# sriram-0311/MC-SLAM

Measured on AMD Instinct MI355X. Metric: multi-cam frames/sec (4-cam 1280x720 @2000 kpts/cam, extract + intra-rig match), higher is better.
Workload: dtype u8; 1 GPU; 4-cam rig 1280x720, 2000 kpts/cam, extract + all-pairs intra-rig match (configs[1]); slots=4, frames_per_launch=128, cameras=4, nfeatures=2000

## Files before the change

### mc-slam_amd/csrc/mcorb_kernels.hip

```cpp
#include <hip/hip_runtime.h>
#include <stdint.h>
#include <string.h>
#include <vector>

#include "mcorb_common.h"
#include "mcorb_device.h"
#include "mcorb_kernels.h"

namespace mcorb {

constexpr int kResizeRows = kResizeTileH;

template <int NF>
__global__ __launch_bounds__(256) void k_resize(uint8_t *__restrict__ pyr, Geom g, int level,
                                                const ResizeTap *__restrict__ tabs, int srcPitch, int srcRows)
{
    extern __shared__ __attribute__((aligned(16))) uint8_t win[];
    const LevelGeom &D = g.lv[level];
    const LevelGeom &S = g.lv[level - 1];
    const int img = blockIdx.z;
    uint8_t *base = pyr + (size_t)img * g.imgBytes;
    const int tid = threadIdx.x;
    const int bx0 = blockIdx.x * 256, by0 = blockIdx.y * kResizeRows;
    const int bx1 = min(bx0 + 255, D.w - 1), by1 = min(by0 + kResizeRows - 1, D.h - 1);
    const int sx0 = tabs[D.xtab + bx0].s0 & ~15, sx1 = tabs[D.xtab + bx1].s1;
    const int sy0 = tabs[D.ytab + by0].s0, sy1 = tabs[D.ytab + by1].s1;
    const int nq = ((sx1 - sx0) >> 4) + 1, nr = sy1 - sy0 + 1;
    const int wave = wave_uniform(tid >> 6);
    const int wy0 = by0 + wave * (kResizeRows / 4);
    uint2 ytap;
    {
        const int l = tid & 63;
        const int dy = min(wy0 + (l < kResizeRows / 4 ? l : 0), D.h - 1);
        ytap = *reinterpret_cast<const uint2 *>(tabs + D.ytab + dy);
    }
    const int dx4 = bx0 + (tid & 63) * 4;
    const int dxc = min(dx4, ((D.w + 3) & ~3) - 4);
    const uint4 t01 = *reinterpret_cast<const uint4 *>(tabs + D.xtab + dxc);
    const uint4 t23 = *reinterpret_cast<const uint4 *>(tabs + D.xtab + dxc + 2);
    {
        const uint8_t *sp = base + S.off + (size_t)sy0 * S.pitch + sx0;
        uint4 *w128 = reinterpret_cast<uint4 *>(win);
        const int pq = srcPitch >> 4;
        const float rcp_pq = 1.0f / (float)pq;
        if constexpr (NF > 0) {
            uint4 v[NF];
            bool ok[NF];
#pragma unroll
            for (int k = 0; k < NF; k++) {
                const int i = tid + 256 * k, ic = min(i, nr * pq - 1);
                const int r = (int)(((float)ic + 0.5f) * rcp_pq), q = ic - r * pq;
                ok[k] = i < nr * pq && q < nq;
                v[k] = *reinterpret_cast<const uint4 *>(sp + (size_t)r * S.pitch + 16 * min(q, nq - 1));
            }
            const int spare = (srcPitch >> 4) * srcRows;
#pragma unroll
            for (int k = 0; k < NF; k++) w128[ok[k] ? tid + 256 * k : spare] = v[k];
        } else {
            for (int i = tid; i < nr * pq; i += 256) {
                const int r = (int)(((float)i + 0.5f) * rcp_pq), q = i - r * pq;
                if (q < nq) w128[i] = *reinterpret_cast<const uint4 *>(sp + (size_t)r * S.pitch + 16 * q);
            }
        }
    }
    __syncthreads();
    asm volatile("" ::"v"(ytap.x), "v"(ytap.y), "v"(t01.x), "v"(t01.y), "v"(t01.z), "v"(t01.w), "v"(t23.x), "v"(t23.y), "v"(t23.z), "v"(t23.w));
    if (dx4 >= D.w) return;
    const uint32_t tw[8] = {t01.x, t01.y, t01.z, t01.w, t23.x, t23.y, t23.z, t23.w};
    int s0[4], s1[4], a0[4], a1[4];
#pragma unroll
    for (int k = 0; k < 4; k++) {
        s0[k] = (int)(tw[2 * k] & 0xffff) - sx0;
        s1[k] = (int)(tw[2 * k] >> 16) - sx0;
        a0[k] = (int)(short)(tw[2 * k + 1] & 0xffff);
        a1[k] = (int)(short)(tw[2 * k + 1] >> 16);
    }
    const uint32_t mask = dx4 + 4 > D.w ? 0xffffffffu >> (8 * (dx4 + 4 - D.w)) : 0xffffffffu;
    int rowA = -1, rowB = -1;
    uint32_t HA[4], HB[4];
    const uint32_t ldsWin = (uint32_t)(uintptr_t)(__attribute__((address_space(3))) void *)win;
    uint32_t sb[4];
#pragma unroll
    for (int k = 0; k < 4; k++) sb[k] = ldsWin + (uint32_t)s0[k];
    auto hrow = [&](int sr, uint32_t *Hout) {
        const uint32_t ro = (uint32_t)__mul24(sr - sy0, srcPitch);
        const uint32_t ad0 = sb[0] + ro, ad1 = sb[1] + ro, ad2 = sb[2] + ro, ad3 = sb[3] + ro;
        uint32_t x0, x1, x2, x3, x4, x5, x6, x7;
        asm volatile("ds_read_u8 %0, %8\n\tds_read_u8 %1, %8 offset:1\n\t"
                     "ds_read_u8 %2, %9\n\tds_read_u8 %3, %9 offset:1\n\t"
                     "ds_read_u8 %4, %10\n\tds_read_u8 %5, %10 offset:1\n\t"
                     "ds_read_u8 %6, %11\n\tds_read_u8 %7, %11 offset:1\n\t"
                     "s_waitcnt lgkmcnt(0)"
                     : "=&v"(x0), "=&v"(x1), "=&v"(x2), "=&v"(x3), "=&v"(x4), "=&v"(x5), "=&v"(x6), "=&v"(x7)
                     : "v"(ad0), "v"(ad1), "v"(ad2), "v"(ad3)
                     : "memory");
        Hout[0] = (__umul24(x0, (uint32_t)a0[0]) + __umul24(x1, (uint32_t)a1[0])) >> 4;
        Hout[1] = (__umul24(x2, (uint32_t)a0[1]) + __umul24(x3, (uint32_t)a1[1])) >> 4;
        Hout[2] = (__umul24(x4, (uint32_t)a0[2]) + __umul24(x5, (uint32_t)a1[2])) >> 4;
        Hout[3] = (__umul24(x6, (uint32_t)a0[3]) + __umul24(x7, (uint32_t)a1[3])) >> 4;
    };
#pragma unroll
    for (int rr = 0; rr < kResizeRows / 4; rr++) {
        const int dy = wy0 + rr;
        if (dy >= D.h) break;
        const uint32_t ys = (uint32_t)__builtin_amdgcn_readlane((int)ytap.x, rr), yc = (uint32_t)__builtin_amdgcn_readlane((int)ytap.y, rr);
        const int r0 = (int)(ys & 0xffff), r1 = (int)(ys >> 16);
        if (r0 != rowA) {
            if (r0 == rowB) {
#pragma unroll
                for (int k = 0; k < 4; k++) HA[k] = HB[k];
            } else {
                hrow(r0, HA);
            }
            rowA = r0;
        }
        if (r1 != rowB) {
            if (r1 == rowA) {
#pragma unroll
                for (int k = 0; k < 4; k++) HB[k] = HA[k];
            } else {
                hrow(r1, HB);
            }
            rowB = r1;
        }
        const uint32_t b0 = yc & 0xffff, b1 = yc >> 16;
        uint32_t p0[4], p1[4];
#pragma unroll
        for (int k = 0; k < 4; k++) {
            p0[k] = __umul24(b0, HA[k]) + 0x20000u;
            p1[k] = __umul24(b1, HB[k]);
        }
        uint32_t t01v, t23v;
        asm("v_add_u32_sdwa %0, %1, %2 dst_sel:DWORD dst_unused:UNUSED_PAD src0_sel:WORD_1 src1_sel:WORD_1" : "=v"(t01v) : "v"(p0[0]), "v"(p1[0]));
        asm("v_add_u32_sdwa %0, %1, %2 dst_sel:WORD_1 dst_unused:UNUSED_PRESERVE src0_sel:WORD_1 src1_sel:WORD_1" : "+v"(t01v) : "v"(p0[1]), "v"(p1[1]));
        asm("v_add_u32_sdwa %0, %1, %2 dst_sel:DWORD dst_unused:UNUSED_PAD src0_sel:WORD_1 src1_sel:WORD_1" : "=v"(t23v) : "v"(p0[2]), "v"(p1[2]));
        asm("v_add_u32_sdwa %0, %1, %2 dst_sel:WORD_1 dst_unused:UNUSED_PRESERVE src0_sel:WORD_1 src1_sel:WORD_1" : "+v"(t23v) : "v"(p0[3]), "v"(p1[3]));
        const u16x2 s01 = __builtin_bit_cast(u16x2, t01v) >> (unsigned short)2, s23 = __builtin_bit_cast(u16x2, t23v) >> (unsigned short)2;
        const uint32_t out = __builtin_amdgcn_perm(__builtin_bit_cast(uint32_t, s23), __builtin_bit_cast(uint32_t, s01), 0x06040200u);
        *reinterpret_cast<uint32_t *>(base + D.off + (size_t)dy * D.pitch + dx4) = out & mask;
    }
}


struct FastCell {
    int on;
    int cell;
    int ph;
    int wi, hi;
    int rows;
    int g0, ng;
    int R;
    float rcp_ng;
    uint32_t headMask, tailMask;
    uint32_t org;
    const uint8_t *src;
    int pitch;
};

constexpr int kFastCellRecDw = 8;
__device__ __forceinline__ void fast_cell_setup(const uint8_t *pyr, const Geom &g, int img, int cell, const uint32_t *__restrict__ rec, FastCell &C)
{
    const uint4 r = *reinterpret_cast<const uint4 *>(rec + (size_t)cell * kFastCellRecDw);
    const uint2 r4 = *reinterpret_cast<const uint2 *>(rec + (size_t)cell * kFastCellRecDw + 4);
    C.cell = cell;
    C.src = pyr + (size_t)img * g.imgBytes + r.x;
    C.org = r.y;
    C.pitch = (int)r.z;
    C.rows = (int)(r.w & 0xff);
    C.wi = (int)((r.w >> 8) & 0xff);
    C.hi = (int)((r.w >> 16) & 0xff);
    C.on = (int)((r.w >> 24) & 1);
    C.ph = (int)((r.w >> 25) & 3);
    C.g0 = (int)(r4.x & 0xff);
    C.ng = (int)((r4.x >> 8) & 0xff);
    C.R = (int)(r4.x >> 16);
    C.rcp_ng = __uint_as_float(r4.y);
    const uint2 r6 = *reinterpret_cast<const uint2 *>(rec + (size_t)cell * kFastCellRecDw + 6);
    C.headMask = r6.x;
    C.tailMask = r6.y;
}

int fast_cell_table(const Geom &g, std::vector<uint32_t> &tab)
{
    const int off = (int)tab.size();
    tab.resize(tab.size() + (size_t)g.cells * kFastCellRecDw, 0u);
    for (int level = 0; level < g.nlevels; level++) {
        const LevelGeom &L = g.lv[level];
        for (int cl = 0; cl < L.nCols * L.nRows; cl++) {
            const int ci = cl / L.nCols, cj = cl - ci * L.nCols;
            const int iniY = kMinBorder + ci * L.hCell;
            int maxY = iniY + L.hCell + 6;
            const int iniX = kMinBorder + cj * L.wCell;
            int maxX = iniX + L.wCell + 6;
            const bool skip = (iniY >= L.maxBorderY - 3) || (iniX >= L.maxBorderX - 6);
            if (maxY > L.maxBorderY) maxY = L.maxBorderY;
            if (maxX > L.maxBorderX) maxX = L.maxBorderX;
            const int cols = maxX - iniX, rows = maxY - iniY;
            const int wi = cols - 6, hi = rows - 6;
            const int ph = iniX & 3, g0 = (ph + 3) >> 2;
            const bool on = !(skip || wi <= 0 || hi <= 0);
            const int ng = on ? ((ph + 2 + wi) >> 2) - g0 + 1 : 1;
            uint32_t *r = tab.data() + off + (size_t)(L.cell0 + cl) * kFastCellRecDw;
            r[0] = on ? (uint32_t)(L.off + (size_t)iniY * L.pitch + (iniX - ph)) : 0u;
            r[1] = ((uint32_t)(ci * L.hCell) << 20) + ((uint32_t)(cj * L.wCell - ph) << 8);
            r[2] = (uint32_t)L.pitch;
            r[3] = on ? ((uint32_t)rows | ((uint32_t)wi << 8) | ((uint32_t)hi << 16) | (1u << 24) | ((uint32_t)ph << 25)) : 0u;
            r[4] = (uint32_t)g0 | ((uint32_t)ng << 8) | ((uint32_t)(64 / ng) << 16);
            const float rcp = 1.0f / (float)ng;
            uint32_t bits;
            memcpy(&bits, &rcp, 4);
            r[5] = bits;
            auto pxmask = [&](int G) {
                static const uint32_t bit[4] = {1u << 15, 1u, 1u << 31, 1u << 16};
                uint32_t m = 0;
                for (int j = 0; j < 4; j++) {
                    const int x = 4 * G + j - (ph + 3);
                    if (x >= 0 && x < wi) m |= bit[j];
                }
                return m;
            };
            r[6] = on ? pxmask(g0) : 0u;
            r[7] = on ? pxmask(g0 + ng - 1) : 0u;
        }
    }
    return off;
}

constexpr int kFastListCap = 768;

#define EMAX __builtin_elementwise_max
#define EMIN __builtin_elementwise_min
struct FastLane {
    int off0;
    uint32_t vmask;
};
template <int TP>
__device__ __forceinline__ FastLane fast_lane_setup(const FastCell &C, int lane)
{
    FastLane L;
    const int r = (int)(((float)lane + 0.5f) * C.rcp_ng);
    const int gi = lane - r * C.ng;
    const bool act = r < C.R;
    L.off0 = act ? (3 + r) * TP + 4 * (C.g0 + gi) : 3 * TP + 4 * C.g0;
    uint32_t m = 0x80018001u;
    m = gi == 0 ? m & C.headMask : m;
    m = gi == C.ng - 1 ? m & C.tailMask : m;
    L.vmask = act ? m : 0u;
    return L;
}

template <int TP>
__device__ __forceinline__ int fast_pass1(const uint8_t *tile, uint32_t *glist, const FastCell &C, int T, int lane, int &row0, int gcap,
                                          const FastLane &L)
{
    const u16x2 Tev = u16x2{(unsigned short)T, (unsigned short)T};
    const u16x2 Tod = u16x2{(unsigned short)(256 * T + 255), (unsigned short)(256 * T + 255)};
    int nG = 0;
    auto trip = [&](int rb, bool tail) {
        int off = L.off0 + rb * TP;
        bool in = true;
        if (tail) {
            in = (int)(((float)lane + 0.5f) * C.rcp_ng) + rb < C.hi;
            off = in ? off : 3 * TP + 4 * C.g0;
        }
        const uint32_t *p = reinterpret_cast<const uint32_t *>(tile + off);
        const uint32_t Cc = p[0], Cl = p[-1], Cr = p[1], Up = p[-3 * (TP / 4)], Dn = p[3 * (TP / 4)];
        const uint32_t Lf = __builtin_amdgcn_alignbyte(Cc, Cl, 1);
        const uint32_t Rt = __builtin_amdgcn_alignbyte(Cr, Cc, 3);
#define U16(X) __builtin_bit_cast(u16x2, (uint32_t)(X))
#define S16(X) __builtin_bit_cast(s16x2, (uint32_t)(X))
        const u16x2 hO = EMIN(EMAX(U16(Up), U16(Dn)), EMAX(U16(Lf), U16(Rt)));
        const u16x2 lO = EMAX(EMIN(U16(Up), U16(Dn)), EMIN(U16(Lf), U16(Rt)));
        const u16x2 hOm = U16(__builtin_bit_cast(uint32_t, hO) & 0xff00ff00u), lOm = U16(__builtin_bit_cast(uint32_t, lO) & 0xff00ff00u);
        const u16x2 vO = U16(Cc & 0xff00ff00u);
        const u16x2 wO = EMAX(__builtin_elementwise_sub_sat(hOm, vO), __builtin_elementwise_sub_sat(vO, lOm));
        const uint32_t zO = __builtin_bit_cast(uint32_t, __builtin_elementwise_sub_sat(wO, Tod));
        const s16x2 vE = S16(Cc & 0x00ff00ffu), uE = S16(Up & 0x00ff00ffu), dE = S16(Dn & 0x00ff00ffu);
        const s16x2 lE = S16(Lf & 0x00ff00ffu), rE = S16(Rt & 0x00ff00ffu);
        const s16x2 wE = EMAX(EMIN(EMAX(uE, dE), EMAX(lE, rE)) - vE, vE - EMAX(EMIN(uE, dE), EMIN(lE, rE)));
        const uint32_t sE = __builtin_bit_cast(uint32_t, __builtin_bit_cast(s16x2, Tev) - wE);
#undef U16
#undef S16
        const uint32_t M = ((sE & 0x80008000u) | (zO & 0x00010001u)) & L.vmask;
        const bool c = M != 0 && in;
        const unsigned long long b = __builtin_amdgcn_ballot_w64(c);
        if (c) glist[lane_rank(b, nG)] = M | ((uint32_t)off >> 1);
        nG += __popcll(b);
    };
    int rb = row0;
    for (; rb + C.R <= C.hi && nG + 64 <= gcap; rb += C.R) trip(rb, false);
    if (rb < C.hi && rb + C.R > C.hi && nG + 64 <= gcap) {
        trip(rb, true);
        rb += C.R;
    }
    row0 = rb;
    return nG;
}

__device__ __forceinline__ int fast_expand(const uint32_t *glist, uint16_t *work, int nG, int lane)
{
    int nA = 0;
    for (int i0 = 0; i0 < nG; i0 += 64) {
        const bool in = i0 + lane < nG;
        const uint32_t E = in ? glist[i0 + lane] : 0u;
        const uint32_t m = E & 0x80018001u;
        const int n1 = in ? __popc(m) - 1 : 0;
        const unsigned long long b0 = __builtin_amdgcn_ballot_w64((n1 & 1) != 0), b1 = __builtin_amdgcn_ballot_w64(n1 >= 2);
        int o = nA + lane + lane_rank(b0) + 2 * lane_rank(b1);
        const uint32_t off = (E & 0x3ffeu) << 1;
        asm volatile("" ::: "memory");
        if (m & 0x8000u) work[o++] = (uint16_t)off;
        if (m & 0x1u) work[o++] = (uint16_t)(off + 1);
        if (m & 0x80000000u) work[o++] = (uint16_t)(off + 2);
        if (m & 0x10000u) work[o++] = (uint16_t)(off + 3);
        const int cnt = min(nG - i0, 64);
        nA += cnt + __popcll(b0) + 2 * __popcll(b1);
        asm volatile("" ::: "memory");
    }
    return nA;
}

template <int TP>
__device__ __forceinline__ int fast_arc_score(const uint8_t *tile, int pos)
{
    int lo = pos - (3 * TP + 3);
    asm volatile("" : "+v"(lo));
    const uint8_t *c = tile + lo + (3 * TP + 3);
    u16x2 X[8];
    X[0] = u16x2{c[3 * TP], c[-3 * TP]};          X[1] = u16x2{c[3 * TP + 1], c[-3 * TP - 1]};
    X[2] = u16x2{c[2 * TP + 2], c[-2 * TP - 2]};  X[3] = u16x2{c[TP + 3], c[-TP - 3]};
    X[4] = u16x2{c[3], c[-3]};                    X[5] = u16x2{c[-TP + 3], c[TP - 3]};
    X[6] = u16x2{c[-2 * TP + 2], c[2 * TP - 2]};  X[7] = u16x2{c[-3 * TP + 1], c[3 * TP - 1]};
    const uint32_t v = c[0];
    u16x2 Sn[8], Sx[8], Pn[8], Px[8];
    Sn[7] = Sx[7] = X[7];
    Pn[0] = Px[0] = X[0];
#pragma unroll
    for (int i = 6; i >= 1; i--) { Sn[i] = EMIN(X[i], Sn[i + 1]); Sx[i] = EMAX(X[i], Sx[i + 1]); }
#pragma unroll
    for (int i = 1; i < 8; i++) { Pn[i] = EMIN(X[i], Pn[i - 1]); Px[i] = EMAX(X[i], Px[i - 1]); }
    Sn[0] = Pn[7]; Sx[0] = Px[7];
    u16x2 bn, bx;
#pragma unroll
    for (int k = 0; k < 8; k++) {
        const u16x2 wn = EMIN(Sn[k], __builtin_shufflevector(Pn[k], Pn[k], 1, 0));
        const u16x2 wx = EMAX(Sx[k], __builtin_shufflevector(Px[k], Px[k], 1, 0));
        bn = k ? EMAX(bn, wn) : wn;
        bx = k ? EMIN(bx, wx) : wx;
    }
    const int Mx = max((int)bn.x, (int)bn.y), Mn = min((int)bx.x, (int)bx.y);
    const int a = max(Mx - (int)v, (int)v - Mn);
    return a < 0 ? 0 : a;
}
#undef EMAX
#undef EMIN

template <int TP>
__global__ __launch_bounds__(64) void k_fast_cells(const uint8_t *__restrict__ pyr, Geom g, int iniTh, int minTh,
                                                   int tileB, int scB, int cap, const uint32_t *__restrict__ cellRec,
                                                   uint32_t *__restrict__ cell_kp, int *__restrict__ cell_cnt)
{
    extern __shared__ __attribute__((aligned(16))) uint8_t lds[];
    constexpr int NQ = TP / 16;
    uint8_t *tile = lds + 16;
    uint8_t *sc = tile + tileB + 16;
    uint8_t *sc2 = sc - 2 * TP;
    uint16_t *work = reinterpret_cast<uint16_t *>(sc + scB + 16);
    uint32_t *glist = reinterpret_cast<uint32_t *>(work + cap / 2);
    const int gcap = cap >> 2;
    struct __attribute__((packed, aligned(4))) Chunk { uint32_t a, b, c, d; };

    const int lane = threadIdx.x;
    const int img = blockIdx.y;
    FastCell C;
    fast_cell_setup(pyr, g, img, wave_uniform(xcd_remap(blockIdx.x, gridDim.x)), cellRec, C);
    int *out_cnt = cell_cnt + (size_t)img * g.cells + C.cell;
    if (!C.on) {
        if (lane == 0) *out_cnt = 0;
        return;
    }

    FastLane FL;
    for (int r = lane; r < C.rows; r += 64) {
        Chunk ch[NQ];
#pragma unroll
        for (int q = 0; q < NQ; q++) ch[q] = *reinterpret_cast<const Chunk *>(C.src + (size_t)r * C.pitch + 16 * q);
        uint4 *dst = reinterpret_cast<uint4 *>(tile + r * TP);
#pragma unroll
        for (int q = 0; q < NQ; q++) dst[q] = uint4{ch[q].a, ch[q].b, ch[q].c, ch[q].d};
    }
    {
        uint4 *s128 = reinterpret_cast<uint4 *>(sc);
        for (int i = lane; i < scB / 16; i += 64) s128[i] = uint4{0, 0, 0, 0};
        FL = fast_lane_setup<TP>(C, lane);
    }
    __syncthreads();

    uint32_t *dst = cell_kp + ((size_t)img * g.cells + C.cell) * g.cellCap;
    int total = 0;
    auto score = [&](int nA, int T) {
        for (int i = lane; i < nA; i += 64) {
            const int pos = work[i];
            const int a = fast_arc_score<TP>(tile, pos);
            sc2[pos] = (uint8_t)(a > T ? a : 0);
        }
    };
    auto nms = [&](int nA) {
        for (int i0 = 0; i0 < nA; i0 += 64) {
            const int i = i0 + lane;
            const int pos = i < nA ? (int)work[i] : 3 * TP;
            int lo = pos - (TP + 1);
            asm volatile("" : "+v"(lo));
            const uint8_t *s = sc2 + lo + (TP + 1);
            const uint32_t a = s[0];
            const uint32_t n = max(max(max((uint32_t)s[1], (uint32_t)s[-1]), max((uint32_t)s[-TP - 1], (uint32_t)s[-TP])),
                                   max(max((uint32_t)s[-TP + 1], (uint32_t)s[TP - 1]), max((uint32_t)s[TP], (uint32_t)s[TP + 1])));
            const bool keep = a > n;
            const unsigned long long b = __builtin_amdgcn_ballot_w64(keep);
            if (keep) {
                const int o = lane_rank(b, total);
                const int yy = (int)(((float)pos + 0.5f) * (1.0f / (float)TP)), xx = __mul24(yy, -TP) + pos;
                if (o < g.cellCap) dst[o] = C.org + ((uint32_t)yy << 20) + ((uint32_t)xx << 8) + (a - 1);
            }
            total += __popcll(b);
        }
    };
    int T = iniTh;
#pragma unroll 1
    for (int attempt = 0; attempt < 2; attempt++) {
        int row0 = 0, sweep = 0;
#pragma unroll 1
        for (;;) {
            const bool whole = row0 == 0;
            const int nG = fast_pass1<TP>(tile, glist, C, T, lane, row0, gcap, FL);
            __syncthreads();
            const int nA = fast_expand(glist, work, nG, lane);
            __syncthreads();
            if (sweep == 0) {
                score(nA, T);
                __syncthreads();
            }
            if (sweep == 1 || (whole && row0 >= C.hi)) nms(nA);
            if (row0 >= C.hi) {
                if (sweep == 1 || whole) break;
                sweep = 1;
                row0 = 0;
            }
            __syncthreads();
        }
        if (total || T == minTh) break;
        T = minTh;
        __syncthreads();
    }
    if (lane == 0) *out_cnt = total;
}

constexpr int kCompactCopies = 4;
template <int kCompactWaves>
__device__ __forceinline__ int block_exclusive_scan(int v, int *wsum, int *total)
{
    const int lane = threadIdx.x & 63, wave = threadIdx.x >> 6;
    int s = v;
#pragma unroll
    for (int o = 1; o < 64; o <<= 1) {
        const int t = __shfl_up(s, o);
        if (lane >= o) s += t;
    }
    if (lane == 63) wsum[wave] = s;
    __syncthreads();
    if (wave == 0) {
        const int w = lane < kCompactWaves ? wsum[lane] : 0;
        int t = w;
#pragma unroll
        for (int o = 1; o < kCompactWaves; o <<= 1) {
            const int u = __shfl_up(t, o);
            if (lane >= o) t += u;
        }
        if (lane < kCompactWaves) wsum[lane] = t - w;
        if (lane == kCompactWaves - 1) *total = t;
    }
    __syncthreads();
    return wsum[wave] + s - v;
}

template <int kCompactWG, int kCompactCells, int NC>
__global__ __launch_bounds__(kCompactWG, 8) void k_compact(const uint32_t *__restrict__ cell_kp, const int *__restrict__ cell_cnt,
                                                        Geom g, const uint16_t *__restrict__ lut, uint32_t *__restrict__ sorted_dev,
                                                        uint32_t *__restrict__ cand, int *__restrict__ tbl,
                                                        int *__restrict__ overflow, int bktCap, int cellsCap)
{
    extern __shared__ __attribute__((aligned(16))) int sh[];
    int *hist = sh;
    uint32_t *bkey = reinterpret_cast<uint32_t *>(hist + NC * bktCap);
    uint16_t *cnts = reinterpret_cast<uint16_t *>(hist + 2 * NC * bktCap);
    constexpr int kCompactWaves = kCompactWG / 64;
    __shared__ int wsum[kCompactWaves];
    __shared__ int s_tot, s_base, s_nz;
    const int tid = threadIdx.x, lane = tid & 63, wave = tid >> 6;
    const int level = blockIdx.y, img = blockIdx.x;
    const LevelGeom &L = g.lv[level];
    const int nc = L.nCols * L.nRows;
    const int *cnt = cell_cnt + (size_t)img * g.cells;
    const int cap = g.cellCap;
    const int B = L.nBuckets;
    const int W0 = L.maxBorderX - kMinBorder, H0 = L.maxBorderY - kMinBorder;
    uint16_t *tx = cnts + cellsCap, *ty = tx + W0;

    int s = 0, t = 0, over = 0;
    for (int c = tid; c < L.cell0; c += kCompactWG) { const int v = cnt[c]; s += v < cap ? v : cap; }
    for (int c = tid; c < nc; c += kCompactWG) {
        int v = cnt[L.cell0 + c];
        if (v > cap) { v = cap; over = 1; }
        cnts[c] = (uint16_t)v;
        t += v;
    }
    for (int c = nc + tid; c < min(nc + 2 * kCompactCells, cellsCap); c += kCompactWG) cnts[c] = 0;
    for (int i = tid; i < W0 + H0; i += kCompactWG) tx[i] = lut[L.lutx + i];
    (void)block_exclusive_scan<kCompactWaves>(s, wsum, &s_base);
    (void)block_exclusive_scan<kCompactWaves>(t, wsum, &s_tot);
    const int base = s_base, T = s_tot;
    for (int b = tid; b < NC * (B + 1); b += kCompactWG) { hist[b] = 0; bkey[b] = 0; }
    int *tb = tbl + (size_t)img * tbl_ints(g.bucketTotal);
    if (tid == 0) {
        s_nz = 0;
        tb[kTblLvlOff + level] = base;
        if (level == g.nlevels - 1) tb[kTblLvlOff + g.nlevels] = base + T;
        if (base + T > g.candCap) over = 1;
    }
    if (over) atomicOr(overflow, 1);
    __syncthreads();

    const uint32_t *src = cell_kp + ((size_t)img * g.cells + L.cell0) * cap;
    const int wave_u = wave_uniform(wave);
    auto walk = [&](auto &&fn) {
        static_assert(kCompactCells == 8 || kCompactCells == 4 || kCompactCells == 2, "the counts are read as one 4-, 8- or 16-byte word");
        constexpr int step = kCompactWaves * kCompactCells;
        const int ncUp = (nc + kCompactCells - 1) & ~(kCompactCells - 1);
        auto load = [&](int c0, int *n, uint32_t *p) {
            if constexpr (kCompactCells == 8) {
                const uint4 q = *reinterpret_cast<const uint4 *>(cnts + c0);
                n[0] = q.x & 0xffff; n[1] = q.x >> 16; n[2] = q.y & 0xffff; n[3] = q.y >> 16;
                n[4] = q.z & 0xffff; n[5] = q.z >> 16; n[6] = q.w & 0xffff; n[7] = q.w >> 16;
            } else if constexpr (kCompactCells == 4) {
                const uint2 q = *reinterpret_cast<const uint2 *>(cnts + c0);
                n[0] = q.x & 0xffff; n[1] = q.x >> 16; n[2] = q.y & 0xffff; n[3] = q.y >> 16;
            } else {
                const uint32_t q = *reinterpret_cast<const uint32_t *>(cnts + c0);
                n[0] = q & 0xffff; n[1] = q >> 16;
            }
#pragma unroll
            for (int u = 0; u < kCompactCells; u++) {
                const uint32_t *cb = src + (size_t)min(c0 + u, nc - 1) * cap;
                p[u] = cb[min(lane, max(n[u], 1) - 1)];
            }
        };
        auto run = [&](int c0, const int *n, const uint32_t *p) {
            int big = 0;
#pragma unroll
            for (int u = 0; u < kCompactCells; u++) {
                big |= n[u];
                if (lane < n[u]) fn(p[u], (c0 + u) * cap + lane);
            }
            if (big > 64) {
#pragma unroll
                for (int u = 0; u < kCompactCells; u++)
                    for (int k = lane + 64; k < n[u]; k += 64) fn(src[(size_t)(c0 + u) * cap + k], (c0 + u) * cap + k);
            }
        };
        int c0 = wave_u * kCompactCells;
        if (c0 >= nc) return;
        int nA[kCompactCells], nB[kCompactCells];
        uint32_t pA[kCompactCells], pB[kCompactCells];
        load(c0, nA, pA);
        while (true) {
            load(min(c0 + step, ncUp), nB, pB);
            run(c0, nA, pA);
            c0 += step;
            if (c0 >= nc) break;
            load(min(c0 + step, ncUp), nA, pA);
            run(c0, nB, pB);
            c0 += step;
            if (c0 >= nc) break;
        }
    };
    walk([&](uint32_t p, int order) {
        const uint32_t code = (uint32_t)tx[cand_x(p)] | (uint32_t)ty[cand_y(p)];
        const uint32_t key = ((uint32_t)cand_resp(p) << 23) | (uint32_t)(kPickOrderMask - order);
        const int slot = (int)code * NC + (lane & (NC - 1));
        atomicAdd(&hist[slot], 1);
        atomicMax(&bkey[slot], key);
    });
    __syncthreads();
    {
        const int bper = (B + kCompactWG - 1) / kCompactWG;
        const int b0 = tid * bper;
        int bs = 0, nzl = 0;
        for (int k = 0; k < bper; k++)
            if (b0 + k < B) {
                int v = 0;
#pragma unroll
                for (int c = 0; c < NC; c++) v += hist[(b0 + k) * NC + c];
                bs += v;
                nzl += v > 0;
            }
        if (nzl) atomicAdd(&s_nz, nzl);
        int brun = block_exclusive_scan<kCompactWaves>(bs, wsum, &s_tot);
        for (int k = 0; k < bper; k++) {
            if (b0 + k < B) {
#pragma unroll
                for (int c = 0; c < NC; c++) { const int v = hist[(b0 + k) * NC + c]; hist[(b0 + k) * NC + c] = brun; brun += v; }
            }
        }
        if (tid == 0) hist[B * NC] = T;
    }
    __syncthreads();
    int *bs_out = tb + kTblHead + L.bucket0;
    for (int b = tid; b <= B; b += kCompactWG) bs_out[b] = hist[b * NC];
    __syncthreads();
    uint32_t *sd = sorted_dev + (size_t)img * g.candCap + base;
    const int room = g.candCap - base;
// ... 452 lines not shown
constexpr int kTileU4 = 4 * 64;
static_assert(32 * kKnnQT * kKnnWaves == kKnnQueriesPerBlock, "the host reads the accepted-pair lists in blocks of kKnnQueriesPerBlock queries");
static_assert(kTileU4 * 16 == 32 * kKnnExpandBytes, "k_expand's tile and the scratch size the engine allocates");

__global__ __launch_bounds__(256) void k_expand(const uint8_t *__restrict__ desc, const int *__restrict__ counts,
                                                const int *__restrict__ setmap, int kcap, uint4 *__restrict__ E,
                                                int *__restrict__ lcounts)
{
    const int i = blockIdx.y;
    const int src = setmap ? setmap[i] : i;
    const int n = min(max(counts[src], 0), kcap);
    if (blockIdx.x == 0 && threadIdx.x == 0) lcounts[i] = n;
    const int d = blockIdx.x * 256 + threadIdx.x;
    if (d >= n) return;
    const uint4 *dp = reinterpret_cast<const uint4 *>(desc + ((size_t)src * kcap + d) * 32);
    const uint4 lo = dp[0], hi = dp[1];
    const uint32_t w[8] = {lo.x, lo.y, lo.z, lo.w, hi.x, hi.y, hi.z, hi.w};
    uint4 *out = E + ((size_t)i * (kcap / 32) + (d >> 5)) * kTileU4 + (d & 31);
#pragma unroll
    for (int sh = 0; sh < 8; sh++) {
        uint32_t o[4];
#pragma unroll
        for (int q = 0; q < 4; q++) {
            uint32_t x = (w[sh] >> (8 * q)) & 0xffu;
            x = (x | (x << 12)) & 0x000f000fu;
            x = (x | (x << 6)) & 0x03030303u;
            x = (x | (x << 3)) & 0x11111111u;
            o[q] = (x << 3) | 0x22222222u;
        }
        out[(sh >> 1) * 64 + (sh & 1) * 32] = uint4{o[0], o[1], o[2], o[3]};
    }
}

template <int kKnnStageTiles, int kWavesPerSimd, bool FOLD>
__global__ __launch_bounds__(64 * kKnnWaves, kWavesPerSimd) void k_knn2(const uint4 *__restrict__ E, const int *__restrict__ lcounts,
                                                           const int2 *__restrict__ pairs, int kcap, int nchunks, int npairs,
                                                           int qblocks, uint2 *__restrict__ part, int chunkLen,
                                                           float dist_thresh, float ratio, KnnRow *__restrict__ rows,
                                                           uint32_t *__restrict__ mlist, int *__restrict__ mcount)
{
    __shared__ __attribute__((aligned(16))) uint4 stage[2 * kKnnStageTiles * kTileU4 + 2 * 64];
    const int tid = threadIdx.x, lane = tid & 63, wave = tid >> 6, half = lane >> 5;
    const int slot = blockIdx.x >> 3, grp = slot / qblocks;
    const int unit = grp * 8 + (blockIdx.x & 7);
    if (unit >= npairs * nchunks) return;
    const int pair = unit / nchunks, chunk = unit - pair * nchunks;
    const int2 qt = pairs[pair];
    const int nq = lcounts[qt.x], nt = lcounts[qt.y];
    const int qbi = slot - grp * qblocks;
    const int qb = qbi * kKnnQueriesPerBlock;
    if (qb >= nq) {
        if (FOLD && tid == 0) mcount[pair * qblocks + qbi] = 0;
        return;
    }
    const int t0 = chunk * chunkLen;
    const int tn = min(nt - t0, chunkLen);
    const int tilesPerSet = kcap / 32;
    const int ntiles = tn > 0 ? (tn + 31) >> 5 : 0;
    const float kNone = -__builtin_inff();
    float k0[kKnnQT], k1[kKnnQT];
#pragma unroll
    for (int u = 0; u < kKnnQT; u++) k0[u] = k1[u] = kNone;

    if (tn > 0) {
        const int qtile0 = (qb >> 5) + wave * kKnnQT;
        v4i Bf[kKnnQT][4];
#pragma unroll
        for (int u = 0; u < kKnnQT; u++) {
            const int tq = min(qtile0 + u, tilesPerSet - 1);
            const uint4 *src = E + ((size_t)qt.x * tilesPerSet + tq) * kTileU4 + lane;
#pragma unroll
            for (int s = 0; s < 4; s++) Bf[u][s] = __builtin_bit_cast(v4i, src[s * 64]);
        }
        v16f Crow;
#pragma unroll
        for (int e = 0; e < 16; e++) Crow[e] = (float)(31 - ((e & 3) + 8 * (e >> 2) + 4 * half));
        const uint4 *Et = E + ((size_t)qt.y * tilesPerSet + (t0 >> 5)) * kTileU4;
        const int nstage = (ntiles + kKnnStageTiles - 1) / kKnnStageTiles;
        static_assert(kTileU4 == 64 * kKnnWaves, "one LDS-DMA round of the workgroup = one tile (wave w moves K-step w)");
        auto fill = [&](int st, int buf) {
#pragma unroll
            for (int k = 0; k < kKnnStageTiles; k++) {
                const int e0 = k * kTileU4 + wave * 64;
                if (st * kKnnStageTiles + k < ntiles)
                    __builtin_amdgcn_global_load_lds((const __attribute__((address_space(1))) void *)(Et + (size_t)st * kKnnStageTiles * kTileU4 + e0 + lane),
                                                     (__attribute__((address_space(3))) void *)(&stage[buf * kKnnStageTiles * kTileU4 + e0]), 16, 0, 0);
            }
        };
        fill(0, 0);
        asm volatile("s_waitcnt vmcnt(0)" ::: "memory");
        __syncthreads();
        auto fold2 = [&](int u, float x, float y) {
            const float t = __builtin_amdgcn_fmed3f(k0[u], x, y);
            k0[u] = __builtin_fmaxf(__builtin_fmaxf(k0[u], x), y);
            k1[u] = __builtin_fmaxf(k1[u], t);
        };
        auto raise = [&]() {
#pragma unroll
            for (int u = 0; u < kKnnQT; u++) { k0[u] += 32.0f; k1[u] += 32.0f; }
        };
        auto top2 = [&](const v16f (&acc)[kKnnQT]) {
            raise();
#pragma unroll
            for (int u = 0; u < kKnnQT; u++)
#pragma unroll
                for (int e = 0; e < 16; e += 2) fold2(u, acc[u][e], acc[u][e + 1]);
        };
        constexpr int kSc = 0x85858585;
        v4i Af[4];
        auto tile = [&](const int base, const uint4 *S, int tb, v16f (&acc)[kKnnQT], const v16f (&old)[kKnnQT]) {
            raise();
#pragma unroll
            for (int s = 0; s < 4; s++) {
                const int g = base + s;
                Af[(g + 2) & 3] = __builtin_bit_cast(v4i, S[(g + 2) * 64 + lane]);
                const v4i a = Af[g & 3];
                const v8i A = {a[0], a[1], a[2], a[3], 0, 0, 0, 0};
#pragma unroll
                for (int u = 0; u < kKnnQT; u++) {
                    const v8i B = {Bf[u][s][0], Bf[u][s][1], Bf[u][s][2], Bf[u][s][3], 0, 0, 0, 0};
                    acc[u] = __builtin_amdgcn_mfma_scale_f32_32x32x64_f8f6f4(A, B, s == 0 ? Crow : acc[u], 4, 4, 0, kSc, 0, kSc);
                }
#pragma unroll
                for (int u = 0; u < kKnnQT; u++) {
                    fold2(u, old[u][4 * s], old[u][4 * s + 1]);
                    fold2(u, old[u][4 * s + 2], old[u][4 * s + 3]);
                }
                __builtin_amdgcn_sched_group_barrier(0x100, 1, 0);
#pragma unroll
                for (int u = 0; u < kKnnQT; u++) {
                    __builtin_amdgcn_sched_group_barrier(0x008, 1, 0);
                    __builtin_amdgcn_sched_group_barrier(0x002, 5, 0);
                }
            }
#pragma unroll
            for (int u = 0; u < kKnnQT; u++) asm volatile("" : "+v"(k0[u]), "+v"(k1[u]));
            if (tb + 32 > tn) {
#pragma unroll
                for (int e = 0; e < 16; e++) {
                    const bool ok = tb + (e & 3) + 8 * (e >> 2) + 4 * half < tn;
#pragma unroll
                    for (int u = 0; u < kKnnQT; u++) acc[u][e] = ok ? acc[u][e] : kNone;
                }
            }
        };
        static_assert(kKnnStageTiles % 2 == 0, "the tile loop walks a stage as pairs of tiles");
        v16f accA[kKnnQT], accB[kKnnQT];
#pragma unroll
        for (int u = 0; u < kKnnQT; u++)
#pragma unroll
            for (int e = 0; e < 16; e++) accA[u][e] = kNone;
        for (int st = 0; st < nstage; st++) {
            if (st + 1 < nstage) fill(st + 1, (st + 1) & 1);
            const uint4 *Sst = stage + (st & 1) * kKnnStageTiles * kTileU4;
            Af[0] = __builtin_bit_cast(v4i, Sst[lane]);
            Af[1] = __builtin_bit_cast(v4i, Sst[64 + lane]);
            const int tcount = min(ntiles - st * kKnnStageTiles, kKnnStageTiles);
#pragma unroll 1
            for (int pr = 0; 2 * pr < tcount; pr++) {
                const uint4 *S = Sst + pr * 2 * kTileU4;
                const int tb0 = (st * kKnnStageTiles + 2 * pr) * 32;
                tile(0, S, tb0, accB, accA);
                if (2 * pr + 1 < tcount) tile(4, S, tb0 + 32, accA, accB);
            }
            asm volatile("s_waitcnt vmcnt(0)" ::: "memory");
            __syncthreads();
        }
        if (ntiles & 1) top2(accB); else top2(accA);
    }
    const int koff = 8160 - 32 * (ntiles - 1) + (1 << 20);
    auto conv = [&](float key) -> uint32_t {
        if (key == kNone) return 0xffffffffu;
        const uint32_t kp = (uint32_t)((int)key + koff);
        return ((256u - (kp >> 13)) << 16) | (uint32_t)(t0 + 8191 - (int)(kp & 8191u));
    };
    if (!FOLD) {
        uint2 *out = part + ((size_t)pair * nchunks + chunk) * kcap;
#pragma unroll
        for (int u = 0; u < kKnnQT; u++) {
            const float o0 = __shfl_xor(k0[u], 32), o1 = __shfl_xor(k1[u], 32);
            const float m0 = fmaxf(k0[u], o0), m1 = fmaxf(fminf(k0[u], o0), fmaxf(k1[u], o1));
            const int q = qb + (wave * kKnnQT + u) * 32 + (lane & 31);
            if (half == 0 && q < nq) out[q] = uint2{conv(m0), conv(m1)};
        }
        return;
    }
    __syncthreads();
    int *wcnt = reinterpret_cast<int *>(&stage[0]);
    uint32_t packed[kKnnQT];
    unsigned long long bal[kKnnQT];
#pragma unroll
    for (int u = 0; u < kKnnQT; u++) {
        const float o0 = __shfl_xor(k0[u], 32), o1 = __shfl_xor(k1[u], 32);
        const float m0 = fmaxf(k0[u], o0), m1 = fmaxf(fminf(k0[u], o0), fmaxf(k1[u], o1));
        const int q = qb + (wave * kKnnQT + u) * 32 + (lane & 31);
        const uint32_t c0 = conv(m0), c1 = conv(m1);
        const bool v0 = c0 != 0xffffffffu, v1 = c1 != 0xffffffffu;
        const uint32_t d0 = v0 ? c0 >> 16 : 0u, d1 = v1 ? c1 >> 16 : 0u, ti0 = c0 & 0xffffu;
        uint32_t acc = 0;
        if (v0 && v1) {
            const float f0 = (float)d0, f1 = (float)d1;
            acc = (f0 < __fmul_rn(ratio, f1)) && !(f0 > dist_thresh);
        }
        const bool mine = half == 0 && q < nq;
        if (mine) {
            KnnRow r;
            r.idx = (v0 ? ti0 : 0xffffu) | ((v1 ? (c1 & 0xffffu) : 0xffffu) << 16);
            r.d = d0 | (d1 << 9) | (acc << 18);
            rows[(size_t)pair * kcap + q] = r;
        }
        bal[u] = __ballot(mine && acc != 0);
        packed[u] = ((uint32_t)q << 16) | ti0;
    }
    if (lane == 0) {
#pragma unroll
        for (int u = 0; u < kKnnQT; u++) wcnt[wave * kKnnQT + u] = __popcll(bal[u]);
    }
    __syncthreads();
    int before = 0;
    for (int i = 0; i < wave * kKnnQT; i++) before += wcnt[i];
    uint32_t *ml = mlist + (size_t)pair * (qblocks * kKnnQueriesPerBlock) + qb;
#pragma unroll
    for (int u = 0; u < kKnnQT; u++) {
        if ((bal[u] >> lane) & 1) ml[lane_rank(bal[u], before)] = packed[u];
        before += __popcll(bal[u]);
    }
    if (wave == kKnnWaves - 1 && lane == 0) mcount[pair * qblocks + qbi] = before;
}

__device__ __forceinline__ void knn_insert(uint32_t key, uint32_t &k0, uint32_t &k1)
{
    const uint32_t hi = key > k0 ? key : k0;
    k1 = hi < k1 ? hi : k1;
    k0 = key < k0 ? key : k0;
}

__global__ __launch_bounds__(1024) void k_knn2_finalize(const uint2 *__restrict__ part, const int *__restrict__ counts,
                                                        const int2 *__restrict__ pairs, int kcap, int nchunks, int chunkLen,
                                                        float dist_thresh, float ratio, KnnRow *__restrict__ out,
                                                        uint32_t *__restrict__ mlist, int *__restrict__ mcount, int qblocks)
{
    __shared__ int wsum[16];
    __shared__ int s_run;
    const int pair = blockIdx.x, tid = threadIdx.x, lane = tid & 63, wave = tid >> 6;
    const int2 qt = pairs[pair];
    const int nq = min(max(counts[qt.x], 0), kcap), nt = min(max(counts[qt.y], 0), kcap);
    const int used = (nt + chunkLen - 1) / chunkLen;
    if (tid == 0) s_run = 0;
    __syncthreads();
    for (int base = 0; base < nq; base += 1024) {
        const int q = base + tid;
        uint32_t acc = 0, t0 = 0;
        if (q < nq) {
            uint32_t k0 = 0xffffffffu, k1 = 0xffffffffu;
            for (int c = 0; c < used; c += 4) {
                uint2 p[4];
#pragma unroll
                for (int u = 0; u < 4; u++)
                    p[u] = c + u < used ? part[((size_t)pair * nchunks + c + u) * kcap + q] : uint2{0xffffffffu, 0xffffffffu};
#pragma unroll
                for (int u = 0; u < 4; u++) {
                    knn_insert(p[u].x, k0, k1);
                    knn_insert(p[u].y, k0, k1);
                }
            }
            const bool v0 = k0 != 0xffffffffu, v1 = k1 != 0xffffffffu;
            const uint32_t d0 = v0 ? k0 >> 16 : 0u, d1 = v1 ? k1 >> 16 : 0u;
            if (v0 && v1) {
                const float f0 = (float)d0, f1 = (float)d1;
                acc = (f0 < __fmul_rn(ratio, f1)) && !(f0 > dist_thresh);
            }
            t0 = k0 & 0xffffu;
            KnnRow r;
            r.idx = (v0 ? t0 : 0xffffu) | ((v1 ? (k1 & 0xffffu) : 0xffffu) << 16);
            r.d = d0 | (d1 << 9) | (acc << 18);
            out[(size_t)pair * kcap + q] = r;
        }
        const unsigned long long b = __ballot(acc != 0);
        if (lane == 0) wsum[wave] = __popcll(b);
        __syncthreads();
        int before = s_run;
        for (int w = 0; w < wave; w++) before += wsum[w];
        if (acc) mlist[(size_t)pair * (qblocks * kKnnQueriesPerBlock) + lane_rank(b, before)] = ((uint32_t)q << 16) | t0;
        __syncthreads();
        if (tid == 0) {
            int tot = 0;
            for (int w = 0; w < 16; w++) tot += wsum[w];
            s_run += tot;
        }
        __syncthreads();
    }
    if (tid < qblocks) mcount[pair * qblocks + tid] = tid == 0 ? s_run : 0;
}

hipError_t upload_umax(const int umax[16]) { return hipMemcpyToSymbol(HIP_SYMBOL(c_umax), umax, 16 * sizeof(int)); }

void launch_pyramid(hipStream_t st, uint8_t *pyr, const Geom &g, const ResizeTap *tabs, const int *win, int nimg)
{
    for (int l = 1; l < g.nlevels; l++) {
        dim3 grid((g.lv[l].w + 255) / 256, (g.lv[l].h + kResizeRows - 1) / kResizeRows, nimg);
        const int srcPitch = win[2 * l], srcRows = win[2 * l + 1];
        const int chunks = (srcPitch >> 4) * srcRows, nf = (chunks + 255) / 256;
        const size_t lds = (size_t)srcPitch * srcRows + 16;
        const auto kern = nf <= 4 ? k_resize<4> : nf <= 8 ? k_resize<8> : k_resize<0>;
        hipLaunchKernelGGL(kern, grid, dim3(256), lds, st, pyr, g, l, tabs, srcPitch, srcRows);
    }
}

void fast_layout(const Geom &g, int &tp, int &rows)
{
    int pitch = 0;
    rows = 0;
    for (int l = 0; l < g.nlevels; l++) {
        const int p = ((3 + g.lv[l].wCell + 6 + 15) >> 4) << 4;
        pitch = pitch > p ? pitch : p;
        rows = rows > g.lv[l].hCell + 6 ? rows : g.lv[l].hCell + 6;
    }
    tp = pitch <= 48 ? 48 : (pitch <= 64 ? 64 : 80);
}

void launch_fast(hipStream_t st, const uint8_t *pyr, const Geom &g, int iniTh, int minTh, const uint32_t *cellRec,
                 uint32_t *cell_kp, int *cell_cnt, int nimg)
{
    int tp, rows;
    fast_layout(g, tp, rows);
    const int cap = kFastListCap;
    const int tileB = (rows * tp + 15) & ~15, scB = ((rows - 4) * tp + 15) & ~15;
    const size_t lds = 16 + (size_t)tileB + 16 + (size_t)scB + 16 + (size_t)cap * 2;
    dim3 grid(g.cells, nimg);
    if (iniTh < 1) iniTh = 1;
    if (minTh < 1) minTh = 1;
    if (iniTh > 255) iniTh = 255;
    if (minTh > 255) minTh = 255;
    const auto kern = tp == 48 ? k_fast_cells<48> : tp == 64 ? k_fast_cells<64> : k_fast_cells<80>;
    hipLaunchKernelGGL(kern, grid, dim3(64), lds, st, pyr, g, iniTh, minTh, tileB, scB, cap, cellRec, cell_kp, cell_cnt);
}

void launch_compact(hipStream_t st, const uint32_t *cell_kp, const int *cell_cnt, const Geom &g, const uint16_t *lut,
                    uint32_t *sorted_dev, uint32_t *cand, int *tbl, int *overflow, int nimg, bool one_copy)
{
    int maxb = 1, maxc = 1, maxwh = 2;
    for (int l = 0; l < g.nlevels; l++) {
        maxb = maxb > g.lv[l].nBuckets ? maxb : g.lv[l].nBuckets;
        maxc = maxc > g.lv[l].nCols * g.lv[l].nRows ? maxc : g.lv[l].nCols * g.lv[l].nRows;
        const int wh = (g.lv[l].maxBorderX - kMinBorder) + (g.lv[l].maxBorderY - kMinBorder);
        maxwh = maxwh > wh ? maxwh : wh;
    }
    const int bktCap = (maxb + 1 + 3) & ~3;
    const int wg = nimg <= 8 ? 1024 : 512;
    const int cellsCap = (maxc + 8 + 7) & ~7;
    const size_t ldsTail = (size_t)(cellsCap + maxwh + 8) * sizeof(uint16_t);
    const bool fits = (size_t)(2 * kCompactCopies * bktCap) * sizeof(int) + ldsTail <= 64 * 1024;
    const int copies = fits && !one_copy ? kCompactCopies : 1;
    const size_t lds = (size_t)(2 * copies * bktCap) * sizeof(int) + ldsTail;
    const dim3 grid(nimg, g.nlevels);
    const auto kern = wg == 1024 ? (copies == 1 ? k_compact<1024, 4, 1> : k_compact<1024, 4, kCompactCopies>)
                                 : (copies == 1 ? k_compact<512, 4, 1> : k_compact<512, 4, kCompactCopies>);
    hipLaunchKernelGGL(kern, grid, dim3(wg), lds, st, cell_kp, cell_cnt, g, lut, sorted_dev, cand, tbl, overflow, bktCap, cellsCap);
}

void launch_blur(hipStream_t st, const uint8_t *pyr, uint8_t *blur, const Geom &g, int nimg)
{
    dim3 grid(g.tiles, nimg);
    hipLaunchKernelGGL(k_blur, grid, dim3(256), 0, st, pyr, blur, g);
}

void launch_describe(hipStream_t st, const uint8_t *pyr, const uint8_t *blur, const Geom &g, const uint32_t *sel,
                     const int *nsel, int orientation, uint8_t *desc, float *angles, int nimg, uint8_t *desc_host)
{
    if (orientation) {
        dim3 grid((g.kcap + 3) / 4, nimg);
        hipLaunchKernelGGL(k_describe_oriented, grid, dim3(256), 0, st, pyr, blur, g, sel, nsel, desc, angles);
    } else {
        dim3 grid((g.kcap + 4 * kDescPerWave - 1) / (4 * kDescPerWave), nimg);
        if (blur) hipLaunchKernelGGL(k_describe, grid, dim3(256), 0, st, blur, g, sel, nsel, desc);
        else hipLaunchKernelGGL(k_describe_fused, dim3(grid.x * nimg), dim3(256), 0, st, pyr, g, sel, nsel, desc, (int)grid.x, desc_host);
    }
}

void launch_knn2(hipStream_t st, const uint8_t *desc, const int *counts, const int *setmap, int nsets, const int2 *pairs, int npairs,
                 int kcap, void *expanded, int *lcounts, uint2 *part, float dist_thresh, float ratio, KnnRow *out, uint32_t *mlist,
                 int *mcount, hipEvent_t ev_exp, hipEvent_t ev_mid)
{
    uint4 *E = reinterpret_cast<uint4 *>(expanded);
    hipLaunchKernelGGL(k_expand, dim3((kcap + 255) / 256, nsets), dim3(256), 0, st, desc, counts, setmap, kcap, E, lcounts);
    if (ev_exp) (void)hipEventRecord(ev_exp, st);
    const int chunkLen = knn_chunk_len(npairs), nchunks = (kcap + chunkLen - 1) / chunkLen;
    const int qblocks = knn_qblocks(kcap), units = npairs * nchunks;
    dim3 grid(8 * qblocks * ((units + 7) / 8));
    if (nchunks == 1) {
        hipLaunchKernelGGL((k_knn2<4, 3, true>), grid, dim3(64 * kKnnWaves), 0, st, E, lcounts, pairs, kcap, nchunks, npairs, qblocks, part, chunkLen,
                           dist_thresh, ratio, out, mlist, mcount);
        if (ev_mid) (void)hipEventRecord(ev_mid, st);
        return;
    }
    hipLaunchKernelGGL((k_knn2<4, 3, false>), grid, dim3(64 * kKnnWaves), 0, st, E, lcounts, pairs, kcap, nchunks, npairs, qblocks, part, chunkLen,
                       dist_thresh, ratio, out, mlist, mcount);
    if (ev_mid) (void)hipEventRecord(ev_mid, st);
    hipLaunchKernelGGL(k_knn2_finalize, dim3(npairs), dim3(1024), 0, st, part, lcounts, pairs, kcap, nchunks, chunkLen, dist_thresh, ratio, out, mlist,
                       mcount, qblocks);
}
}
```

Before: 40520 frames/s.

## Swizzle resize block order across images and streamline pyramid and FAST expand

The resize kernel remaps block indices so that groups of 8 images interleave their tiles, which is meant to improve cache locality and spread load across the device. It also precomputes the reciprocal pitch on the host, simplifies source-offset arithmetic with 24-bit multiplies, ping-pongs the cached horizontal rows, and uses explicit mad/mul instructions with scalar operands. Separately, fast_expand replaces its branchy per-bit stores with a lookup table of slot positions and four unconditional ds_write_b16 stores, removing divergence. The unconditional writes rely on the work buffer having slack past the end, and the tile remap relies on the magic-number division being exact.

```diff
diff --git a/mc-slam_amd/csrc/mcorb_kernels.hip b/mc-slam_amd/csrc/mcorb_kernels.hip
--- a/mc-slam_amd/csrc/mcorb_kernels.hip
+++ b/mc-slam_amd/csrc/mcorb_kernels.hip
@@ -13,18 +13,27 @@
 
 template <int NF>
 __global__ __launch_bounds__(256) void k_resize(uint8_t *__restrict__ pyr, Geom g, int level,
-                                                const ResizeTap *__restrict__ tabs, int srcPitch, int srcRows)
+                                                const ResizeTap *__restrict__ tabs, int srcPitch, int srcRows, float rcpPq, int rowMagic)
 {
     extern __shared__ __attribute__((aligned(16))) uint8_t win[];
     const LevelGeom &D = g.lv[level];
     const LevelGeom &S = g.lv[level - 1];
-    const int img = blockIdx.z;
+    const int tid = threadIdx.x;
+    int tx = blockIdx.x, ty = blockIdx.y, img = blockIdx.z;
+    if (rowMagic && img < (int)(gridDim.z & ~7u)) {
+        const int m = tx + (int)gridDim.x * ty + (int)(gridDim.x * gridDim.y) * (img & 7);
+        const int t = m >> 3;
+        img = (img & ~7) | (m & 7);
+        ty = (t * rowMagic) >> 16;
+        tx = t - ty * (int)gridDim.x;
+    }
     uint8_t *base = pyr + (size_t)img * g.imgBytes;
-    const int tid = threadIdx.x;
-    const int bx0 = blockIdx.x * 256, by0 = blockIdx.y * kResizeRows;
+    const int bx0 = tx * 256, by0 = ty * kResizeRows;
     const int bx1 = min(bx0 + 255, D.w - 1), by1 = min(by0 + kResizeRows - 1, D.h - 1);
-    const int sx0 = tabs[D.xtab + bx0].s0 & ~15, sx1 = tabs[D.xtab + bx1].s1;
-    const int sy0 = tabs[D.ytab + by0].s0, sy1 = tabs[D.ytab + by1].s1;
+    const uint32_t cx0 = *reinterpret_cast<const uint32_t *>(tabs + D.xtab + bx0), cx1 = *reinterpret_cast<const uint32_t *>(tabs + D.xtab + bx1);
+    const uint32_t cy0 = *reinterpret_cast<const uint32_t *>(tabs + D.ytab + by0), cy1 = *reinterpret_cast<const uint32_t *>(tabs + D.ytab + by1);
+    const int sx0 = (int)(cx0 & 0xfff0u), sx1 = (int)(cx1 >> 16);
+    const int sy0 = (int)(cy0 & 0xffffu), sy1 = (int)(cy1 >> 16);
     const int nq = ((sx1 - sx0) >> 4) + 1, nr = sy1 - sy0 + 1;
     const int wave = wave_uniform(tid >> 6);
     const int wy0 = by0 + wave * (kResizeRows / 4);
@@ -42,24 +51,26 @@
         const uint8_t *sp = base + S.off + (size_t)sy0 * S.pitch + sx0;
         uint4 *w128 = reinterpret_cast<uint4 *>(win);
         const int pq = srcPitch >> 4;
-        const float rcp_pq = 1.0f / (float)pq;
+        const int rowStep = S.pitch - srcPitch;
+        const float f0 = (float)tid + 0.5f;
         if constexpr (NF > 0) {
             uint4 v[NF];
             bool ok[NF];
 #pragma unroll
             for (int k = 0; k < NF; k++) {
-                const int i = tid + 256 * k, ic = min(i, nr * pq - 1);
-                const int r = (int)(((float)ic + 0.5f) * rcp_pq), q = ic - r * pq;
-                ok[k] = i < nr * pq && q < nq;
-                v[k] = *reinterpret_cast<const uint4 *>(sp + (size_t)r * S.pitch + 16 * min(q, nq - 1));
+                const int i = tid + 256 * k;
+                const int r = (int)((f0 + (float)(256 * k)) * rcpPq), q = i - __mul24(r, pq);
+                ok[k] = r < nr && q < nq;
+                const uint32_t off = (uint32_t)(__mul24(r, rowStep) + 16 * i);
+                v[k] = *reinterpret_cast<const uint4 *>(sp + (ok[k] ? off : 0u));
             }
             const int spare = (srcPitch >> 4) * srcRows;
 #pragma unroll
             for (int k = 0; k < NF; k++) w128[ok[k] ? tid + 256 * k : spare] = v[k];
         } else {
             for (int i = tid; i < nr * pq; i += 256) {
-                const int r = (int)(((float)i + 0.5f) * rcp_pq), q = i - r * pq;
-                if (q < nq) w128[i] = *reinterpret_cast<const uint4 *>(sp + (size_t)r * S.pitch + 16 * q);
+                const int r = (int)(((float)i + 0.5f) * rcpPq), q = i - __mul24(r, pq);
+                if (q < nq) w128[i] = *reinterpret_cast<const uint4 *>(sp + (uint32_t)(__mul24(r, rowStep) + 16 * i));
             }
         }
     }
@@ -67,21 +78,17 @@
     asm volatile("" ::"v"(ytap.x), "v"(ytap.y), "v"(t01.x), "v"(t01.y), "v"(t01.z), "v"(t01.w), "v"(t23.x), "v"(t23.y), "v"(t23.z), "v"(t23.w));
     if (dx4 >= D.w) return;
     const uint32_t tw[8] = {t01.x, t01.y, t01.z, t01.w, t23.x, t23.y, t23.z, t23.w};
-    int s0[4], s1[4], a0[4], a1[4];
+    uint32_t a0[4], a1[4];
 #pragma unroll
     for (int k = 0; k < 4; k++) {
-        s0[k] = (int)(tw[2 * k] & 0xffff) - sx0;
-        s1[k] = (int)(tw[2 * k] >> 16) - sx0;
-        a0[k] = (int)(short)(tw[2 * k + 1] & 0xffff);
-        a1[k] = (int)(short)(tw[2 * k + 1] >> 16);
+        a0[k] = tw[2 * k + 1] & 0xffffu;
+        a1[k] = tw[2 * k + 1] >> 16;
     }
     const uint32_t mask = dx4 + 4 > D.w ? 0xffffffffu >> (8 * (dx4 + 4 - D.w)) : 0xffffffffu;
-    int rowA = -1, rowB = -1;
-    uint32_t HA[4], HB[4];
     const uint32_t ldsWin = (uint32_t)(uintptr_t)(__attribute__((address_space(3))) void *)win;
     uint32_t sb[4];
 #pragma unroll
-    for (int k = 0; k < 4; k++) sb[k] = ldsWin + (uint32_t)s0[k];
+    for (int k = 0; k < 4; k++) sb[k] = ldsWin + (tw[2 * k] & 0xffffu) - (uint32_t)sx0;
     auto hrow = [&](int sr, uint32_t *Hout) {
         const uint32_t ro = (uint32_t)__mul24(sr - sy0, srcPitch);
         const uint32_t ad0 = sb[0] + ro, ad1 = sb[1] + ro, ad2 = sb[2] + ro, ad3 = sb[3] + ro;
@@ -94,17 +101,21 @@
                      : "=&v"(x0), "=&v"(x1), "=&v"(x2), "=&v"(x3), "=&v"(x4), "=&v"(x5), "=&v"(x6), "=&v"(x7)
                      : "v"(ad0), "v"(ad1), "v"(ad2), "v"(ad3)
                      : "memory");
-        Hout[0] = (__umul24(x0, (uint32_t)a0[0]) + __umul24(x1, (uint32_t)a1[0])) >> 4;
-        Hout[1] = (__umul24(x2, (uint32_t)a0[1]) + __umul24(x3, (uint32_t)a1[1])) >> 4;
-        Hout[2] = (__umul24(x4, (uint32_t)a0[2]) + __umul24(x5, (uint32_t)a1[2])) >> 4;
-        Hout[3] = (__umul24(x6, (uint32_t)a0[3]) + __umul24(x7, (uint32_t)a1[3])) >> 4;
+        Hout[0] = (__umul24(x0, a0[0]) + __umul24(x1, a1[0])) >> 4;
+        Hout[1] = (__umul24(x2, a0[1]) + __umul24(x3, a1[1])) >> 4;
+        Hout[2] = (__umul24(x4, a0[2]) + __umul24(x5, a1[2])) >> 4;
+        Hout[3] = (__umul24(x6, a0[3]) + __umul24(x7, a1[3])) >> 4;
     };
+    int held[2] = {-1, -1};
+    uint32_t H[2][4];
 #pragma unroll
     for (int rr = 0; rr < kResizeRows / 4; rr++) {
         const int dy = wy0 + rr;
         if (dy >= D.h) break;
         const uint32_t ys = (uint32_t)__builtin_amdgcn_readlane((int)ytap.x, rr), yc = (uint32_t)__builtin_amdgcn_readlane((int)ytap.y, rr);
         const int r0 = (int)(ys & 0xffff), r1 = (int)(ys >> 16);
+        uint32_t(&HA)[4] = H[(rr & 1) ^ 1], (&HB)[4] = H[rr & 1];
+        int &rowA = held[(rr & 1) ^ 1], &rowB = held[rr & 1];
         if (r0 != rowA) {
             if (r0 == rowB) {
 #pragma unroll
@@ -125,10 +136,11 @@
         }
         const uint32_t b0 = yc & 0xffff, b1 = yc >> 16;
         uint32_t p0[4], p1[4];
+        const uint32_t half = 0x20000u;
 #pragma unroll
         for (int k = 0; k < 4; k++) {
-            p0[k] = __umul24(b0, HA[k]) + 0x20000u;
-            p1[k] = __umul24(b1, HB[k]);
+            asm("v_mad_u32_u24 %0, %1, %2, %3" : "=v"(p0[k]) : "v"(HA[k]), "s"(b0), "v"(half));
+            asm("v_mul_u32_u24_e32 %0, %1, %2" : "=v"(p1[k]) : "s"(b1), "v"(HB[k]));
         }
         uint32_t t01v, t23v;
         asm("v_add_u32_sdwa %0, %1, %2 dst_sel:DWORD dst_unused:UNUSED_PAD src0_sel:WORD_1 src1_sel:WORD_1" : "=v"(t01v) : "v"(p0[0]), "v"(p1[0]));
@@ -297,8 +309,27 @@
     return nG;
 }
 
+struct FastExpandTab { uint32_t t0, t1, t2; };
+constexpr FastExpandTab fast_expand_tab()
+{
+    FastExpandTab T{0, 0, 0};
+    for (uint32_t i = 0; i < 16; i++) {
+        const bool set[4] = {(i & 1) != 0, (i & 8) != 0, (i & 4) != 0, (i & 2) != 0};
+        uint32_t place[4] = {0, 0, 0, 0};
+        int n = 0;
+        for (uint32_t j = 0; j < 4; j++)
+            if (set[j]) place[n++] = j;
+        T.t0 |= place[0] << (2 * i);
+        T.t1 |= place[1] << (2 * i);
+        T.t2 |= place[2] << (2 * i);
+    }
+    return T;
+}
+static_assert(kFastListCap % 256 == 0, "fast_expand: cap / 4 must be a multiple of the 64 groups of a trip");
 __device__ __forceinline__ int fast_expand(const uint32_t *glist, uint16_t *work, int nG, int lane)
 {
+    constexpr FastExpandTab T = fast_expand_tab();
+    const uint32_t ldsWork = (uint32_t)(uintptr_t)(__attribute__((address_space(3))) void *)work;
     int nA = 0;
     for (int i0 = 0; i0 < nG; i0 += 64) {
         const bool in = i0 + lane < nG;
@@ -306,16 +337,23 @@
         const uint32_t m = E & 0x80018001u;
         const int n1 = in ? __popc(m) - 1 : 0;
         const unsigned long long b0 = __builtin_amdgcn_ballot_w64((n1 & 1) != 0), b1 = __builtin_amdgcn_ballot_w64(n1 >= 2);
-        int o = nA + lane + lane_rank(b0) + 2 * lane_rank(b1);
+        const int cnt = min(nG - i0, 64);
+        const int end = nA + cnt + __popcll(b0) + 2 * __popcll(b1);
+        const int o = min(nA + lane + lane_rank(b0) + 2 * lane_rank(b1), end);
         const uint32_t off = (E & 0x3ffeu) << 1;
+        const uint32_t rot = __builtin_amdgcn_alignbit(m, m, 15);
+        const uint32_t sh = (rot << 1) | (rot >> 13);
+        const uint32_t d0 = off | __builtin_amdgcn_ubfe(T.t0, sh, 2u), d1 = off | __builtin_amdgcn_ubfe(T.t1, sh, 2u);
+        const uint32_t d2 = off | __builtin_amdgcn_ubfe(T.t2, sh, 2u), d3 = off | 3u;
         asm volatile("" ::: "memory");
-        if (m & 0x8000u) work[o++] = (uint16_t)off;
-        if (m & 0x1u) work[o++] = (uint16_t)(off + 1);
-        if (m & 0x80000000u) work[o++] = (uint16_t)(off + 2);
-        if (m & 0x10000u) work[o++] = (uint16_t)(off + 3);
-        const int cnt = min(nG - i0, 64);
-        nA += cnt + __popcll(b0) + 2 * __popcll(b1);
-        asm volatile("" ::: "memory");
+        asm volatile("ds_write_b16 %0, %4 offset:6\n\t"
+                     "ds_write_b16 %0, %3 offset:4\n\t"
+                     "ds_write_b16 %0, %2 offset:2\n\t"
+                     "ds_write_b16 %0, %1"
+                     :
+                     : "v"(ldsWork + 2u * (uint32_t)o), "v"(d0), "v"(d1), "v"(d2), "v"(d3)
+                     : "memory");
+        nA = end;
     }
     return nA;
 }
@@ -1374,8 +1412,10 @@
         const int srcPitch = win[2 * l], srcRows = win[2 * l + 1];
         const int chunks = (srcPitch >> 4) * srcRows, nf = (chunks + 255) / 256;
         const size_t lds = (size_t)srcPitch * srcRows + 16;
+        const float rcpPq = 1.0f / (float)(srcPitch >> 4);
+        const int rowMagic = grid.x <= 16 && grid.x * grid.y <= 2048 ? (int)((65536 + grid.x - 1) / grid.x) : 0;
         const auto kern = nf <= 4 ? k_resize<4> : nf <= 8 ? k_resize<8> : k_resize<0>;
-        hipLaunchKernelGGL(kern, grid, dim3(256), lds, st, pyr, g, l, tabs, srcPitch, srcRows);
+        hipLaunchKernelGGL(kern, grid, dim3(256), lds, st, pyr, g, l, tabs, srcPitch, srcRows, rcpPq, rowMagic);
     }
 }
 
```

Result: faster. 41150 frames/s (median of 5 runs) (+1.6%).
